# microsoft/MoGe

Hardware: AMD Instinct MI355X
Metric: images/sec (MoGeModel.infer, moge-2-vitl 518x518 fp16) (higher is better)
Workload: dtype f16; 1 GPU; moge-2-vitl infer(): batch 32/GPU x 3x518x518 torch.rand, num_tokens 3600, fp16 weights, synthetic checkpoint (seed 0), inputs resident in HBM, outputs left on device; global_batch=32, parallelism=dp1 (independent shards, one-time RCCL weight broadcast)

## Files before the change

include/moge_hip.h:

```cpp
#ifndef MOGE_HIP_H
#define MOGE_HIP_H

#include <stddef.h>
#include <stdint.h>

#ifdef __cplusplus
extern "C" {
#endif

#define MOGE_ABI_VERSION 5
#define MOGE_MAX_TAPS 8
#define MOGE_LEVELS 5

typedef enum moge_status {
    MOGE_OK = 0,
    MOGE_ERR_INVALID = -1,
    MOGE_ERR_HIP = -2,
    MOGE_ERR_NOT_LOADED = -3,
    MOGE_ERR_MISSING_KEY = -4,
    MOGE_ERR_NONFINITE = -5
} moge_status;

typedef enum moge_precision {
    MOGE_FP32 = 0,
// ... 158 lines not shown
int moge_test_attention(int precision, const float* q, const float* k, const float* v, float* o, int B, int nh, int N, void* stream);
int moge_test_conv3x3(int precision, const float* x, const float* w, const float* bias, float* y, int B, int H, int W,
                      int Cin, int Cout, int relu_in, void* stream);
typedef struct moge_test_conv_args {
    int32_t precision, B, H, W, Cin, Cout;
    int32_t relu_in, act, up2;
    const float* x; const float* w; const float* bias;
    const float* add;
    const float* side; const float* side_w;
    const float* wu; const float* wv; float u0, u1, v0, v1;
    const float* w2; const float* bias2;
    float* y;
    const float* dot_w; int32_t dot_rows;
} moge_test_conv_args;
int moge_test_conv_ex(const moge_test_conv_args* args, void* stream);
typedef struct moge_test_ct3_args {
    int32_t precision, B, H, W, Cin, Cout, no_border;
    const float* x; const float* wt; const float* bt; const float* w3; const float* b3;
    const float* side; const float* side_w;
    const float* wu; const float* wv; float u0, u1, v0, v1;
    float* y;
} moge_test_ct3_args;
int moge_test_ct3(const moge_test_ct3_args* args, void* stream);
int moge_test_convt2x2(int precision, const float* x, const float* w, const float* bias, float* y, int B, int H, int W,
                       int Cin, int Cout, void* stream);
int moge_test_preprocess(const float* image, float* out, int B, int H, int W, int rows, int cols, void* stream);
int moge_test_preprocess_ex(int in_fp16, int out_fp16, const float* image, float* out, int32_t* zero_i32, int B, int H, int W, int rows, int cols, int ldk,
                            int nchw_out, int round16, int aa, int zero_n, void* stream);
int moge_test_resize_bicubic_aa(const float* image, float* out, int B, int H, int W, int OH, int OW, void* stream);
int moge_test_resize_bicubic_aa_ex(int in_fp16, const float* image, float* out, int B, int H, int W, int OH, int OW, int round16, void* stream);
int moge_test_groupnorm_relu(int precision, const float* x, const float* gamma, const float* beta, float* y, int B, int H, int W, int C, int groups, void* stream);
int moge_test_norm_act(int precision, const float* x, const float* gamma, const float* beta, float* y, int B, int H, int W, int C, int groups, int act, int in_place, void* stream);
int moge_test_posembed(const float* pos, float* out, int D, int rows, int cols, void* stream);
int moge_test_posembed_ex(const float* pos, float* out, int D, int rows, int cols, int size_mode, void* stream);
int moge_test_recover(const float* points, const uint8_t* mask, const float* focal_in, int B, int H, int W,
                      float* focal, float* shift, int32_t* status, void* stream);
typedef struct moge_test_head_args {
    int32_t precision, kind, remap, ksize;
    int32_t B, Hd, Wd, C, ld, choff, H, W;
    int32_t n4_below;
    const float* x; const float* w; const float* bias;
    const float* n4; const float* w2;
    float* out;
} moge_test_head_args;
int moge_test_head_final(const moge_test_head_args* args, void* stream);
int moge_test_head_final_dot(int kind, int remap, const float* y, const float* z, int zld, int zoff, const float* bias, float* out, int B, int Hd, int Wd,
// ... 185 lines not shown
```

moge_amd/_lib.py:

```python
from __future__ import annotations

import ctypes as C
import os

import torch

HERE = os.path.dirname(os.path.abspath(__file__))
LIB_PATH = os.path.join(HERE, "lib", "libmoge_hip.so")
EXPERIMENTS_LIB_PATH = os.path.join(HERE, "lib", "experiments", "libmoge_hip.so")

MOGE_MAX_TAPS = 8
MOGE_LEVELS = 5
FP32, FP16, FP16_HALF = 0, 1, 2
HEAD_POINTS, HEAD_NORMAL, HEAD_MASK, HEAD_SCALE = 1, 2, 4, 8
FORCE_PROJECTION, APPLY_MASK = 1, 2
REMAP = {"linear": 0, "sinh": 1, "exp": 2, "sinh_exp": 3}
RESAMPLER = {"conv_transpose": 0, "bilinear": 1, "nearest": 2, "pixel_shuffle": 3}
RES_NORM = {"none": 0, "layer_norm": 1, "group_norm": 2, "instance_norm": 3}
ACTIVATION = {"relu": 0, "leaky_relu": 1, "silu": 2, "elu": 3}
ERR_NONFINITE = -5
KC_NAMES = ["gemm", "attn", "conv", "norm", "pre", "post", "recover", "gemm_pp"]
ABI_VERSION = 5
MESH_MAX_MAPS, MESH_BLOCK_PX, MESH_SCAN_SPAN, MESH_NO_FACES = 8, 1024, 256, -1
MESH_F32, MESH_U8, MESH_UV = 0, 1, 2
# ... 96 lines not shown
    "moge_set_onnx_compatible_mode": (C.c_int, [_vp, _i32]),
    "moge_workspace_bytes": (C.c_int, [_vp, _i32, _i32, _i32, _i32, _i32, C.POINTER(C.c_size_t)]),
    "moge_forward": (C.c_int, [_vp, _vp, _i32, _i32, _i32, _i32, _i32, _i32, C.POINTER(Outputs), _vp]),
    "moge_infer": (C.c_int, [_vp, _vp, _i32, _i32, _i32, _i32, _i32, _i32, _vp, _i32, C.POINTER(Outputs), _vp]),
    "moge_postprocess": (C.c_int, [_vp, _vp, _vp, _vp, _vp, _i32, _i32, _i32, _vp, _i32, C.POINTER(Outputs), _vp]),
    "moge_depth_edge_mask": (C.c_int, [_vp, _vp, _vp, _i32, _i32, _i32, C.c_float, _vp, _vp]),
    "moge_cast_f16": (C.c_int, [_vp, _vp, C.c_int64, _vp]),
    "moge_sync": (C.c_int, [_vp, _vp]),
    "moge_profile_enable": (C.c_int, [_vp, _i32]),
    "moge_profile_read": (C.c_int, [_vp, C.POINTER(Profile), _i32]),
    "moge_debug_tap": (C.c_int, [_vp, C.c_char_p, _vp, _i64, C.POINTER(_i64), _vp]),
    "moge_tune_set": (C.c_int, [C.c_char_p, _i32]),
    "moge_tune_reset": (C.c_int, [C.c_char_p]),
    "moge_tune_value": (C.c_int, [C.c_char_p, C.POINTER(C.c_int)]),
    "moge_test_gemm": (C.c_int, [_i32, _f32p, _f32p, _f32p, _f32p, _i32, _i32, _i32, _i32, _vp]),
    "moge_test_gemm_ex": (C.c_int, [C.POINTER(TestGemmArgs), _vp]),
    "moge_test_gemm_fused_ln": (C.c_int, [_f32p, _f32p, _f32p, _f32p, _f32p, _f32p, _f32p, _f32p, _vp, _i32, _i32, _i32, _vp]),
    "moge_test_layernorm": (C.c_int, [_i32, _f32p, _f32p, _f32p, _f32p, _i32, _i32, _vp]),
    "moge_test_attention": (C.c_int, [_i32, _f32p, _f32p, _f32p, _f32p, _i32, _i32, _i32, _vp]),
    "moge_test_conv3x3": (C.c_int, [_i32, _f32p, _f32p, _f32p, _f32p, _i32, _i32, _i32, _i32, _i32, _i32, _vp]),
    "moge_test_conv_ex": (C.c_int, [C.POINTER(TestConvArgs), _vp]),
    "moge_test_convt2x2": (C.c_int, [_i32, _f32p, _f32p, _f32p, _f32p, _i32, _i32, _i32, _i32, _i32, _vp]),
    "moge_test_ct3": (C.c_int, [C.POINTER(TestCt3Args), _vp]),
    "moge_test_preprocess": (C.c_int, [_f32p, _f32p, _i32, _i32, _i32, _i32, _i32, _vp]),
    "moge_test_preprocess_ex": (C.c_int, [_i32, _i32, _f32p, _f32p, _vp, _i32, _i32, _i32, _i32, _i32, _i32, _i32, _i32, _i32, _i32, _vp]),
    "moge_test_resize_bicubic_aa": (C.c_int, [_f32p, _f32p, _i32, _i32, _i32, _i32, _i32, _vp]),
    "moge_test_resize_bicubic_aa_ex": (C.c_int, [_i32, _f32p, _f32p, _i32, _i32, _i32, _i32, _i32, _i32, _vp]),
    "moge_test_groupnorm_relu": (C.c_int, [_i32, _f32p, _f32p, _f32p, _f32p, _i32, _i32, _i32, _i32, _i32, _vp]),
    "moge_test_norm_act": (C.c_int, [_i32, _f32p, _f32p, _f32p, _f32p, _i32, _i32, _i32, _i32, _i32, _i32, _i32, _vp]),
    "moge_test_posembed": (C.c_int, [_f32p, _f32p, _i32, _i32, _i32, _vp]),
    "moge_test_posembed_ex": (C.c_int, [_f32p, _f32p, _i32, _i32, _i32, _i32, _vp]),
    "moge_test_recover": (C.c_int, [_f32p, _vp, _f32p, _i32, _i32, _i32, _f32p, _f32p, _vp, _vp]),
    "moge_test_head_final": (C.c_int, [C.POINTER(TestHeadArgs), _vp]),
    "moge_test_head_final_dot": (C.c_int, [_i32, _i32, _f32p, _f32p, _i32, _i32, _f32p, _f32p, _i32, _i32, _i32, _i32, _i32, _vp]),
    "moge_test_mlp_layer": (C.c_int, [_f32p, _f32p, _f32p, _f32p, _i32, _i32, _i32, _i32, _vp]),
    "moge_test_layernorm_ex": (C.c_int, [_i32, _i32, _f32p, _f32p, _f32p, _f32p, _f32p, _i32, _i32, _i32, _i32, _i32, _i32, _vp]),
    "moge_test_ln_raw": (C.c_int, [_f32p, _f32p, _f32p, _i32, _i32, _vp]),
    "moge_test_ln_finalize": (C.c_int, [_f32p, _f32p, _i32, _i32, _i32, _vp]),
    "moge_test_fold_ln": (C.c_int, [_f32p, _f32p, _f32p, _f32p, _f32p, _f32p, _f32p, _i32, _i32, _vp]),
    "moge_test_resize_bilinear_uv": (C.c_int, [_i32, _f32p, _f32p, _i32, _i32, _i32, _i32, _i32, _i32, _i32, C.c_float, C.c_float, C.c_float, C.c_float, _vp]),
    "moge_test_u8_ingest": (C.c_int, [_i32, _vp, _f32p, _i32, _i32, _i32, _vp]),
    "moge_align_l1": (C.c_int, [_f32p, _f32p, _f32p, _i32, _i32, C.c_float, _f32p, _f32p, _vp, _vp]),
    "moge_align_l1_anchored": (C.c_int, [_f32p, _f32p, _f32p, _i32, _i32, _i32, _vp, _vp, _i32, C.c_float, _f32p, _f32p, _vp, _vp]),
    "moge_align_trunc_workspace": (C.c_int, [_i32, _i32, C.POINTER(_i64)]),
    "moge_align_trunc": (C.c_int, [_f32p, _f32p, _f32p, _i32, _i32, C.c_float, C.c_float, _vp, _f32p, _f32p, _vp, _vp]),
    "moge_align_trunc_anchored": (C.c_int, [_f32p, _f32p, _f32p, _i32, _i32, _i32, _vp, _vp, _i32, C.c_float, C.c_float, _vp, _f32p, _f32p, _vp, _vp]),
# ... 197 lines not shown
```

moge_amd/csrc/common.h:

```cpp
#pragma once
#include <hip/hip_runtime.h>
#include <stdint.h>
#include <stddef.h>
#include "../../include/moge_hip.h"

typedef _Float16 f16;
typedef unsigned int u32x4 __attribute__((ext_vector_type(4)));
typedef unsigned int u32x2 __attribute__((ext_vector_type(2)));
typedef f16 f16x8 __attribute__((ext_vector_type(8)));
typedef f16 f16x4 __attribute__((ext_vector_type(4)));
typedef f16 f16x2 __attribute__((ext_vector_type(2)));
typedef float f32x2 __attribute__((ext_vector_type(2)));
typedef float f32x4 __attribute__((ext_vector_type(4)));
typedef float f32x16 __attribute__((ext_vector_type(16)));

template <typename T> struct TT;
template <> struct TT<f16> {
    static constexpr int CH = 8;
    static constexpr int PREC = 1;
};
template <> struct TT<float> {
    static constexpr int CH = 4;
    static constexpr int PREC = 0;
};
// ... 194 lines not shown
    static int cus[64] = {};
    int dev = 0;
    if (hipGetDevice(&dev) != hipSuccess) return 256;
    if (dev >= 0 && dev < 64 && cus[dev]) return cus[dev];
    hipDeviceProp_t p;
    const int n = (hipGetDeviceProperties(&p, dev) == hipSuccess && p.multiProcessorCount > 0) ? p.multiProcessorCount : 256;
    if (dev >= 0 && dev < 64) cus[dev] = n;
    return n;
}

template <typename T> int launch_gemm(const GemmArgs& g, int amode, hipStream_t st);
bool gemm_pp_eligible(const GemmArgs& g);
int moge_internal_fail(int code, const char* fmt, ...) __attribute__((format(printf, 2, 3)));
inline int launched(const char* what) {
    const hipError_t e = hipGetLastError();
    return e == hipSuccess ? 0 : moge_internal_fail(MOGE_ERR_HIP, "%s (%s)", what, hipGetErrorString(e));
}
inline unsigned blocks(int64_t n, int per) { return (unsigned)((n + per - 1) / per); }
bool gemm_fuses_ln_finalize(const GemmArgs& g);
bool gemm_runs_pp(const GemmArgs& g);
int launch_gemm_pp(const GemmArgs& g, hipStream_t st);
bool conv_pp_eligible(const GemmArgs& g);
int launch_conv_pp(const GemmArgs& g, hipStream_t st);
struct Ct3Slot { int rowblk, colblk, nterms; int term[13]; };
int launch_ct3_combine(const float* P, const Ct3Slot* slots_dev, int nslots, int Cout, int Cin, void* out, int ld, hipStream_t st);
int launch_ct3_border(const void* in, const void* dw, void* out, int B, int H, int W, int Cin, int Cout, hipStream_t st);
bool conv_rb_eligible(const GemmArgs& g);
int launch_conv_rb(const GemmArgs& g, hipStream_t st);
#include "tune.h"
```

moge_amd/csrc/conv_pp.hip:

```cpp
#include "common.h"

#define CP_GPTR(p) ((const __attribute__((address_space(1))) void*)(p))
__device__ __forceinline__ unsigned cp_opaque(unsigned v) { asm volatile("" : "+v"(v)); return v; }
#define CP_LPTR(p) ((__attribute__((address_space(3))) void*)(p))

namespace {

template <int TW> struct Halo {
    static constexpr int W = TW + 2;
    static constexpr int PX = 18 * W;
    static constexpr int PIECES = (PX + 7) / 8;
    static constexpr int BYTES = PIECES * 1024;
    static constexpr int HPW = (PIECES + 7) / 8;
};

__device__ __forceinline__ u32x4 relu8(u32x4 v) {
#pragma unroll
    for (int i = 0; i < 4; i++) {
        unsigned t = v[i];
        asm("v_pk_max_f16 %0, %0, 0" : "+v"(t));
        v[i] = t;
    }
    return v;
}

template <int N> __device__ __forceinline__ void wait_vm_lgkm() { asm volatile("s_waitcnt vmcnt(%0) lgkmcnt(0)" ::"n"(N) : "memory"); }

template <int BN, int TW, int NH, int EPI>
__global__ __launch_bounds__(512, (BN == 64 && TW == 16 && NH == 1) ? 4 : 2) void conv_pp_kernel(const GemmArgs g) {
    constexpr bool CONVT = (EPI & 2) != 0, HAS_UV = (EPI & 1) != 0, RELU_IN = (EPI & 4) != 0;
    constexpr bool M16 = (EPI & 8) != 0;
    static_assert(!M16 || TW == 16, "16x16x32 path: 16-pixel-wide tiles");
    constexpr bool SIDE_REG = (EPI & 16) != 0;
    constexpr bool DOT = (EPI & 32) != 0;
    static_assert(!DOT || (CONVT && M16 && BN == 128), "fused output conv: the 64 -> 4 x 32 pixel-shuffle resampler");
    constexpr bool CT3 = (EPI & 64) != 0;
    static_assert(!CT3 || (CONVT && M16 && !DOT && !RELU_IN && !SIDE_REG && NH == 2), "fused ConvTranspose2d + 3x3: pixel-shuffle store, 16x16x32 form, two halo buffers");
    constexpr int NTAP = CT3 ? 4 : 9;
    static_assert(!SIDE_REG || (M16 && BN == 64 && NH == 1), "register side input: single-image 64-channel form");
    constexpr int WN = BN / 64, WM = 8 / WN, TM = TW * 16 / 32 / WM, TN = 2;
    constexpr int HALO_W = Halo<TW>::W, HALO_PX = Halo<TW>::PX, HALO_PIECES = Halo<TW>::PIECES, HALO_BYTES = Halo<TW>::BYTES, HPW = Halo<TW>::HPW;
    constexpr int LOG_TW = TW == 16 ? 4 : 5;
    constexpr bool PERSIST = !(BN == 64 && NH == 1);
    constexpr int NWP = BN / 64;
    constexpr int WSLOT = BN * 128;
    constexpr int LDS_W = NH * HALO_BYTES;
    constexpr int WROWS = TM * 32;
    extern __shared__ __attribute__((aligned(16))) char smem[];

    const int tid = threadIdx.x, lane = tid & 63;
    const int wave = __builtin_amdgcn_readfirstlane(tid >> 6);
    const int grp = wave >> 2;
    const int hi = lane >> 5, l31 = lane & 31;
    const int wm = wave / WN, wn = wave % WN;

    const int H = g.H, W = g.W, C = g.C;
    const int tx_n = (W + TW - 1) / TW, ty_n = (H + 15) >> 4;
    const int nbn = g.N / BN;
    int li, cnt, start, wgs_x;
    {
        const int nwg = gridDim.x;
        const int ntiles = PERSIST ? (g.M / (H * W)) * ty_n * tx_n * nbn : nwg;
        const int nx = nwg < 8 ? nwg : 8, xcd = blockIdx.x % nx;
        const int q = ntiles / nx, r = ntiles % nx;
        cnt = q + (xcd < r ? 1 : 0);
        start = xcd * q + min(xcd, r);
        wgs_x = (nwg - xcd + nx - 1) / nx;
        li = blockIdx.x / nx;
    }
    if (li >= cnt) return;
    int b, y0, x0, n0;
    const int nchunks = NH == 1 ? 1 : (C >> 6);
    const int C2 = CT3 ? g.Cout : C;
    const int nside = SIDE_REG ? 1 : ((NH > 1 && g.a2) ? (C2 >> 6) : 0);
    const int nkt1 = nchunks * NTAP;
    const int nkt = nkt1 + nside;

    const int prow = lane >> 3, pch = lane & 7;
    const char* in_b;
    const char* in2_b;
    const char* w_b;
    const char* w2_b;
    unsigned hoff[HPW];
    unsigned hoff2[CT3 ? HPW : 1];
    int sb, sy0, sx0, sn0;
    auto setup = [&](int idx) {
        int prow_t = prow, pch_t = pch;
        if constexpr (PERSIST) asm volatile("" : "+v"(prow_t), "+v"(pch_t));
        const int wgt = start + idx;
        const int bn_ = wgt % nbn;
        int t = wgt / nbn;
        const int tx = t % tx_n; t /= tx_n;
        const int ty = t % ty_n;
        sb = t / ty_n; sy0 = ty * 16; sx0 = tx * TW; sn0 = bn_ * BN;
        in_b = reinterpret_cast<const char*>(g.a) + (size_t)sb * H * W * C * 2;
        in2_b = reinterpret_cast<const char*>(g.a2) + (size_t)sb * H * W * C2 * (CT3 ? 8 : 2);
        w_b = reinterpret_cast<const char*>(g.w) + (size_t)sn0 * g.ldw * 2;
        w2_b = reinterpret_cast<const char*>(g.w2) + (CT3 ? (size_t)0 : (size_t)sn0 * C * 2);
        const int spy = CT3 ? (sn0 / BN) >> 1 : 0, spx = CT3 ? (sn0 / BN) & 1 : 0;
#pragma unroll
        for (int i = 0; i < HPW; i++) {
            int piece = wave + 8 * i;
            piece = piece < HALO_PIECES ? piece : HALO_PIECES - 1;
            int hp = piece * 8 + prow_t;
            const int sw = ((EPI & 8) ? (hp % HALO_W) : ((hp % HALO_W) >> 1)) & 7;
            hp = hp < HALO_PX ? hp : HALO_PX - 1;
            const int hy = hp / HALO_W, hx = hp - hy * HALO_W;
            int yy = sy0 - 1 + hy, xx = sx0 - 1 + hx;
            yy = yy < 0 ? 0 : (yy > H - 1 ? H - 1 : yy);
            xx = xx < 0 ? 0 : (xx > W - 1 ? W - 1 : xx);
            hoff[i] = (unsigned)(((yy * W + xx) * C) * 2 + ((pch_t ^ sw) << 4));
            if constexpr (CT3) hoff2[i] = (unsigned)((((2 * yy + spy) * (2 * W) + 2 * xx + spx) * C2) * 2 + ((pch_t ^ sw) << 4));
        }
    };
    int wrow[NWP];
    unsigned wsw[NWP];
#pragma unroll
    for (int i = 0; i < NWP; i++) {
        wrow[i] = (wave + 8 * i) * 8 + prow;
        wsw[i] = (unsigned)((pch ^ ((wrow[i] >> 1) & 7)) << 4);
    }
    auto issue_halo = [&](int c) {
        char* dst = smem + (c & (NH - 1)) * HALO_BYTES;
        const char* src = uniform_ptr(c < nchunks ? in_b + (size_t)c * 128 : in2_b + (size_t)(c - nchunks) * 128);
        const bool side2 = CT3 && c >= nchunks;
#pragma unroll
        for (int i = 0; i < HPW; i++) {
            int piece = wave + 8 * i;
            piece = piece < HALO_PIECES ? piece : HALO_PIECES - 1;
            unsigned off = hoff[i];
            if constexpr (CT3) off = side2 ? hoff2[i] : off;
            __builtin_amdgcn_global_load_lds(CP_GPTR(src + cp_opaque(off)), CP_LPTR(dst + piece * 1024), 16, 0, 0);
        }
    };
    auto issue_w = [&](int kt) {
        char* dst = smem + LDS_W + (kt & 3) * WSLOT;
        const bool side = kt >= nkt1;
        const int c = CT3 ? kt >> 2 : kt / 9, tap = CT3 ? kt & 3 : kt - c * 9;
        const char* src = uniform_ptr(side ? w2_b + (size_t)(kt - nkt1) * 128 : w_b + ((size_t)tap * C + c * 64) * 2);
        const int rowb = side ? C2 * 2 : g.ldw * 2;
#pragma unroll
        for (int i = 0; i < NWP; i++) {
            const unsigned off = (unsigned)(wrow[i] * rowb) + wsw[i];
            __builtin_amdgcn_global_load_lds(CP_GPTR(src + cp_opaque(off)), CP_LPTR(dst + (wave + 8 * i) * 1024), 16, 0, 0);
        }
    };

    int hp0[TM], hx0[TM];
#pragma unroll
    for (int i = 0; i < TM; i++) {
        const int mp = wm * WROWS + i * 32 + l31;
        hx0[i] = (mp & (TW - 1)) + 1;
        hp0[i] = ((mp >> LOG_TW) + 1) * HALO_W + hx0[i];
    }
    const int sxw = (l31 >> 1) & 7;
    const int w_off = (wn * 64 + l31) * 128 + ((hi ^ sxw) << 4);
    const int l15 = lane & 15, g4 = lane >> 4;
    const int w_off16 = (wn * 64 + l15) * 128 + ((g4 ^ ((l15 >> 1) & 7)) << 4);

    f32x16 acc[TM][TN];
    f32x4 acc16[2 * TM][4];
    const int ntot = nchunks + nside;
    int kt = 0, halo_age = 2;
    int l15t = l15;
    int abase[3][2];
    int tpy = 0;
    auto set_abase = [&]() {
        const bool ph2 = CT3 && BN == 2 * g.Cout;
        const int tpx = CT3 ? (ph2 ? wn : (n0 / BN) & 1) : 0;
        if constexpr (CT3) tpy = ph2 ? (n0 / BN) & 1 : (n0 / BN) >> 1;
#pragma unroll
        for (int d = 0; d < 3; d++) {
            const int hx = l15t + (CT3 ? (d == 2 ? 1 : tpx + d) : d);
            const int a = wm * (2 * TM * HALO_W * 128) + hx * 128 + ((g4 ^ (hx & 7)) << 4);
            abase[d][0] = a; abase[d][1] = a ^ 64;
        }
    };
    u32x4 sidef[SIDE_REG ? 2 * TM : 1][2];
    auto kstep = [&](const char* halo, int dy, int dx, bool first_of_image, int image, bool relu, bool from_regs = false) {
        const char* wsl = smem + LDS_W + (kt & 3) * WSLOT;
        u32x4 af[TM][4], wf[TN][4];
        if constexpr (M16) {
            if (from_regs) {
                if constexpr (SIDE_REG) {
#pragma unroll
                    for (int i = 0; i < 2 * TM; i++)
#pragma unroll
                        for (int ks = 0; ks < 2; ks++) af[i >> 1][(i & 1) * 2 + ks] = sidef[i][ks];
                }
            } else {
#pragma unroll
            for (int i = 0; i < 2 * TM; i++) {
#pragma unroll
                for (int ks = 0; ks < 2; ks++)
                    af[i >> 1][(i & 1) * 2 + ks] = *reinterpret_cast<const u32x4*>(halo + abase[dx + 1][ks] + (i + 1 + dy) * (HALO_W * 128));
            }
            }
#pragma unroll
            for (int j = 0; j < 4; j++)
#pragma unroll
                for (int ks = 0; ks < 2; ks++) wf[j >> 1][(j & 1) * 2 + ks] = *reinterpret_cast<const u32x4*>(wsl + (w_off16 ^ (ks * 64)) + j * 2048);
        } else {
#pragma unroll
        for (int i = 0; i < TM; i++) {
            const int hp = hp0[i] + dy * HALO_W + dx;
// ... 5 lines not shown
        for (int j = 0; j < TN; j++)
#pragma unroll
            for (int ks = 0; ks < 4; ks++) wf[j][ks] = *reinterpret_cast<const u32x4*>(wsl + (w_off ^ (ks * 32)) + j * 4096);
        }
        const bool halo_now = NH > 1 && first_of_image && image + 1 < ntot;
        if (halo_now) { issue_halo(image + 1); halo_age = 0; }
        const int ahead = nkt - 2 - kt;
        if (ahead >= 2) issue_w(kt + 3);
        if (halo_now && image >= nchunks) {
            if (ahead >= 2) wait_vm_lgkm<NWP>();
            else wait_vm_lgkm<0>();
        } else if (NH > 1 && halo_age <= 1) {
            if (ahead >= 2) wait_vm_lgkm<2 * NWP + HPW>();
            else if (ahead == 1) wait_vm_lgkm<NWP + HPW>();
            else wait_vm_lgkm<HPW>();
        } else {
            if (ahead >= 2) wait_vm_lgkm<2 * NWP>();
            else if (ahead == 1) wait_vm_lgkm<NWP>();
            else wait_vm_lgkm<0>();
        }
        halo_age++;
        if constexpr (RELU_IN) {
            if (relu) {
#pragma unroll
                for (int i = 0; i < TM; i++)
#pragma unroll
                    for (int ks = 0; ks < 4; ks++) af[i][ks] = relu8(af[i][ks]);
            }
        }
        __builtin_amdgcn_s_barrier();
        asm volatile("" ::: "memory");
        __builtin_amdgcn_sched_barrier(0);
        __builtin_amdgcn_s_setprio(1);
        if constexpr (M16) {
#pragma unroll
            for (int ks = 0; ks < 2; ks++)
#pragma unroll
                for (int i = 0; i < 2 * TM; i++)
#pragma unroll
                    for (int j = 0; j < 4; j++) mma16<f16>(acc16[i][j], wf[j >> 1][(j & 1) * 2 + ks], af[i >> 1][(i & 1) * 2 + ks]);
        } else {
#pragma unroll
        for (int ks = 0; ks < 4; ks++)
#pragma unroll
            for (int i = 0; i < TM; i++)
#pragma unroll
                for (int j = 0; j < TN; j++) mma_step<f16>(acc[i][j], wf[j][ks], af[i][ks]);
        }
        __builtin_amdgcn_s_setprio(0);
        __builtin_amdgcn_sched_barrier(0);
        asm volatile("" ::: "memory");
        if (!(grp == 1 && kt == nkt - 1)) __builtin_amdgcn_s_barrier();
        asm volatile("" ::: "memory");
        __builtin_amdgcn_sched_barrier(0);
        kt++;
    };
    setup(li);
    if constexpr (SIDE_REG) {
#pragma unroll
        for (int i = 0; i < 2 * TM; i++) {
            int y = sy0 + wm * 2 * TM + i, x = sx0 + l15;
            y = y < H ? y : H - 1; x = x < W ? x : W - 1;
            const char* sp = in2_b + ((size_t)y * W + x) * C * 2 + g4 * 16;
#pragma unroll
            for (int ks = 0; ks < 2; ks++) sidef[i][ks] = *reinterpret_cast<const u32x4*>(sp + ks * 64);
        }
    }
    issue_halo(0);
    bool first = true;
    for (;;) {
    b = sb; y0 = sy0; x0 = sx0; n0 = sn0;
    if constexpr (PERSIST) { asm volatile("" : "+v"(l15t)); if constexpr (M16) set_abase(); }
    else if constexpr (M16) set_abase();
#pragma unroll
    for (int i = 0; i < TM; i++)
#pragma unroll
        for (int j = 0; j < TN; j++)
#pragma unroll
            for (int r = 0; r < 16; r++) acc[i][j][r] = 0.f;
#pragma unroll
    for (int i = 0; i < 2 * TM; i++)
#pragma unroll
        for (int j = 0; j < 4; j++) acc16[i][j] = f32x4{0.f, 0.f, 0.f, 0.f};

    if (!first) {
        asm volatile("s_waitcnt lgkmcnt(0)" ::: "memory");
        __builtin_amdgcn_s_barrier();
        asm volatile("" ::: "memory");
    }
    first = false;
    kt = 0; halo_age = 2;
    issue_w(0);
    issue_w(1);
    issue_w(2);
    wait_vm_lgkm<2 * NWP>();
    __builtin_amdgcn_s_barrier();
    if (grp == 1) __builtin_amdgcn_s_barrier();
    asm volatile("" ::: "memory");
    __builtin_amdgcn_sched_barrier(0);

    for (int c = 0; c < nchunks; c++) {
        const char* halo = smem + (c & (NH - 1)) * HALO_BYTES;
        if constexpr (CT3) {
            const char* hp = halo + tpy * (HALO_W * 128);
#pragma unroll
            for (int tap = 0; tap < 4; tap++) kstep(hp, (tap >> 1) - 1, (tap & 1) - 1, tap == 0, c, true);
        } else {
#pragma unroll
        for (int tap = 0; tap < 9; tap++) kstep(halo, tap / 3 - 1, tap % 3 - 1, tap == 0, c, true);
        }
    }
    if constexpr (SIDE_REG) kstep(smem, 0, 0, false, nchunks, false, true);
    else
    for (int c2 = 0; c2 < nside; c2++) kstep(smem + ((nchunks + c2) & (NH - 1)) * HALO_BYTES, 0, CT3 ? 1 : 0, true, nchunks + c2, false);

    char* R = smem + (PERSIST ? LDS_W : 0) + wave * (WROWS * 128);
    int rr = lane >> 3, cc = lane & 7;
    if constexpr (PERSIST) asm volatile("" : "+v"(rr), "+v"(cc));
    const int nw = n0 + wn * 64;
    const float lo = g.act == ACT_RELU ? 0.f : -3.0e38f;
    const bool has_bias = g.bias != nullptr;
    f16* const outp = reinterpret_cast<f16*>(g.out);
    const f16* const addp = reinterpret_cast<const f16*>(g.add);
    f16x8 addv[WROWS / 8];
    auto load_skip_rows = [&]() {
        if constexpr (!CONVT) {
            if (addp) {
    #pragma unroll
                for (int it = 0; it < WROWS / 8; it++) {
                    const int mp = wm * WROWS + it * 8 + rr;
                    int y = y0 + (mp >> LOG_TW), x = x0 + (mp & (TW - 1));
                    y = y < H ? y : H - 1; x = x < W ? x : W - 1;
                    addv[it] = *reinterpret_cast<const f16x8*>(addp + (((size_t)b * H + y) * W + x) * g.ldadd + nw + cc * 8);
                }
            }
        }
    };
    if constexpr (PERSIST) load_skip_rows();
    u32x4 dota[DOT ? 3 : 1], dotb[DOT ? 2 * TM : 1][2];
    if constexpr (DOT) {
#pragma unroll
        for (int gq = 0; gq < 3; gq++)
            dota[gq] = *reinterpret_cast<const u32x4*>(reinterpret_cast<const char*>(g.dot_tab) + (gq < g.dot_nd ? gq : 0) * 1024 + lane * 16);
    }
    if constexpr (M16) {
        float u0[2 * TM], u1[2 * TM], v0[2 * TM], v1[2 * TM];
        if constexpr (HAS_UV) {
#pragma unroll
            for (int i = 0; i < 2 * TM; i++) {
                int y = y0 + wm * 2 * TM + i, x = x0 + l15;
                y = y < H ? y : H - 1; x = x < W ? x : W - 1;
                if constexpr (CONVT) {
                    u0[i] = linspace_at(g.uv.u0, g.uv.u1, g.uv.ustep, 2 * W, 2 * x);
                    u1[i] = linspace_at(g.uv.u0, g.uv.u1, g.uv.ustep, 2 * W, 2 * x + 1);
                    v0[i] = linspace_at(g.uv.v0, g.uv.v1, g.uv.vstep, 2 * H, 2 * y);
                    v1[i] = linspace_at(g.uv.v0, g.uv.v1, g.uv.vstep, 2 * H, 2 * y + 1);
                } else {
                    u0[i] = u1[i] = linspace_at(g.uv.u0, g.uv.u1, g.uv.ustep, W, x);
                    v0[i] = v1[i] = linspace_at(g.uv.v0, g.uv.v1, g.uv.vstep, H, y);
                }
            }
        }
        f32x4 bvs[4];
#pragma unroll
        for (int jj = 0; jj < 4; jj++) bvs[jj] = *reinterpret_cast<const f32x4*>(g.bias + nw + jj * 16 + 4 * g4);
#pragma unroll
        for (int jj = 0; jj < 4; jj++) {
            const int n = nw + jj * 16 + 4 * g4;
            const f32x4 bv = bvs[jj];
            f32x4 wu = {0.f, 0.f, 0.f, 0.f}, wv = wu;
            int pdy = 0, pdx = 0;
            if constexpr (HAS_UV) {
                int nco = n;
                if constexpr (CONVT) { const int qd = n / g.Cout; nco = n - qd * g.Cout; pdy = qd >> 1; pdx = qd & 1; }
                wu = *reinterpret_cast<const f32x4*>(g.uv.wu + nco);
                wv = *reinterpret_cast<const f32x4*>(g.uv.wv + nco);
            }
#pragma unroll
            for (int i = 0; i < 2 * TM; i++) {
                const int row = i * 16 + l15;
                float v[4];
#pragma unroll
                for (int e = 0; e < 4; e++) v[e] = acc16[i][jj][e] + bv[e];
                if constexpr (HAS_UV) {
                    const float uu = pdx ? u1[i] : u0[i];
                    const float vq = pdy ? v1[i] : v0[i];
#pragma unroll
                    for (int e = 0; e < 4; e++) v[e] += wu[e] * uu + wv[e] * vq;
                }
#pragma unroll
                for (int e = 0; e < 4; e++) v[e] = fmaxf(v[e], lo);
                const f16x4 hv = {(f16)v[0], (f16)v[1], (f16)v[2], (f16)v[3]};
                if constexpr (DOT) {
                    const u32x2 hw = __builtin_bit_cast(u32x2, hv);
                    dotb[i][jj >> 1][(jj & 1) * 2] = hw[0];
                    dotb[i][jj >> 1][(jj & 1) * 2 + 1] = hw[1];
                } else {
                    *reinterpret_cast<f16x4*>(R + row * 128 + ((((jj * 2 + (g4 >> 1)) ^ (row & 7)) << 4) | ((g4 & 1) << 3))) = hv;
                }
            }
        }
        if constexpr (DOT) {
            float* const dout = g.dot_out;
            const int nd4 = 4 * g.dot_nd;
#pragma unroll
            for (int i = 0; i < 2 * TM; i++) {
                const int y = y0 + wm * 2 * TM + i, x = x0 + l15;
                const bool mine = g4 == i && y < H && x < W;
#pragma unroll
                for (int p = 0; p < 2; p++) {
                    const size_t px = ((size_t)b * 2 * H + 2 * y + wn) * (2 * W) + 2 * x + p;
#pragma unroll
                    for (int gq = 0; gq < 3; gq++)
                        if (gq < g.dot_nd) {
                            f32x4 d = {0.f, 0.f, 0.f, 0.f};
                            mma16<f16>(d, dota[gq], dotb[i][p]);
                            if (mine) *reinterpret_cast<f32x4*>(dout + px * nd4 + 4 * gq) = d;
                        }
                }
            }
        }
    } else {
    float u0[TM], u1[TM], v0[TM], v1[TM];
    if constexpr (HAS_UV) {
#pragma unroll
        for (int i = 0; i < TM; i++) {
            const int mp = wm * WROWS + i * 32 + l31;
            int y = y0 + (mp >> LOG_TW), x = x0 + (mp & (TW - 1));
            y = y < H ? y : H - 1; x = x < W ? x : W - 1;
            if constexpr (CONVT) {
                u0[i] = linspace_at(g.uv.u0, g.uv.u1, g.uv.ustep, 2 * W, 2 * x);
// ... 32 lines not shown
                    const float vq = pdy ? v1[i] : v0[i];
#pragma unroll
                    for (int e = 0; e < 4; e++) v[e] += wu[e] * uu + wv[e] * vq;
                }
#pragma unroll
                for (int e = 0; e < 4; e++) v[e] = fmaxf(v[e], lo);
                const f16x4 hv = {(f16)v[0], (f16)v[1], (f16)v[2], (f16)v[3]};
                *reinterpret_cast<f16x4*>(R + row * 128 + ((((j * 4 + q) ^ (row & 7)) << 4) | (hi << 3))) = hv;
            }
        }
    }
    if constexpr (!PERSIST) load_skip_rows();
    bool more = false;
    if constexpr (PERSIST) {
        li += wgs_x;
        more = li < cnt;
        if (more) setup(li);
        __builtin_amdgcn_s_waitcnt(0x0F70);
        if (more) issue_halo(0);
        asm volatile("" ::: "memory");
    }
    if constexpr (!DOT)
#pragma unroll
    for (int it = 0; it < WROWS / 8; it++) {
        const int row = it * 8 + rr;
        const int mp = wm * WROWS + row;
        const int y = y0 + (mp >> LOG_TW), x = x0 + (mp & (TW - 1));
        u32x4 v = *reinterpret_cast<const u32x4*>(R + row * 128 + ((cc ^ (row & 7)) << 4));
        if (y < H && x < W) {
            if constexpr (CONVT) {
                const int n = nw + cc * 8;
                const int qd = n / g.Cout, co = n - qd * g.Cout, pdy = qd >> 1, pdx = qd & 1;
                const size_t idx = ((((size_t)b * 2 * H + 2 * y + pdy) * (2 * W)) + 2 * x + pdx) * g.Cout + co;
                *reinterpret_cast<u32x4*>(outp + idx) = v;
            } else {
                const size_t idx = (((size_t)b * H + y) * W + x) * g.ldc + nw + cc * 8;
                if (addp) {
                    f16x8 h = __builtin_bit_cast(f16x8, v);
                    h += addv[it];
                    v = __builtin_bit_cast(u32x4, h);
                }
                *reinterpret_cast<u32x4*>(outp + idx) = v;
            }
        }
    }
    if (!more) break;
    }
}

template <int BN, int TW, int NH, int EPI>
int launch_conv_cfg(const GemmArgs& g, hipStream_t st) {
    constexpr int smem = NH * Halo<TW>::BYTES + 4 * BN * 128;
    constexpr auto kern = conv_pp_kernel<BN, TW, NH, EPI>;
    if (int rc = set_dyn_lds<kern>(smem)) return rc;
    const long B = (long)g.M / ((long)g.H * g.W);
    const long tiles = B * ((g.H + 15) / 16) * ((g.W + TW - 1) / TW) * (g.N / BN);
    const int ncu = pp_device_cus();
    long slots = (BN == 64 && NH == 1) ? tiles : (long)ncu;
    const long cap = moge_tune_get(TK_CONV_GRID);
    if (cap > 0 && !(BN == 64 && NH == 1)) slots = cap;
    const long grid = tiles < slots ? tiles : slots;
    hipLaunchKernelGGL(kern, dim3((unsigned)grid), dim3(512), smem, st, g);
    return (int)hipGetLastError();
}

}

bool conv_pp_eligible(const GemmArgs& g) {
    if (g.ct3) {
        if ((g.C & 63) || g.K != 4 * g.C || g.ldw != 4 * g.C || !g.bias || g.epi != EPI_CONVT || g.N != 4 * g.Cout) return false;
        if (g.Cout != 128 && g.Cout != 64) return false;
        if (g.add || g.act != ACT_NONE || g.relu_in || g.dot_tab || (g.a2 && !g.w2)) return false;
        if (g.a2 && g.Cout == 64) return false;
        if (g.H < 1 || g.W < 1 || (long)g.M % ((long)g.H * g.W) != 0) return false;
        if ((long)g.H * g.W * g.C * 2 >= (1L << 31) || (long)g.H * g.W * g.Cout * 8 >= (1L << 31)) return false;
// ... 109 lines not shown
            const f32x4 p = red[w][j][lane];
#pragma unroll
            for (int e = 0; e < 4; e++) acc[j][e] += p[e];
        }
    if (!valid) return;
    f16* op = out + (((size_t)b * 2 * H + Y) * (2 * W) + X) * Cout + 4 * g4;
#pragma unroll
    for (int j = 0; j < NJ; j++) {
        f16x4 v = *reinterpret_cast<const f16x4*>(op + j * 16);
        v = f16x4{(f16)((float)v[0] + acc[j][0]), (f16)((float)v[1] + acc[j][1]), (f16)((float)v[2] + acc[j][2]), (f16)((float)v[3] + acc[j][3])};
        *reinterpret_cast<f16x4*>(op + j * 16) = v;
    }
}

int launch_ct3_border(const void* in, const void* dw, void* out, int B, int H, int W, int Cin, int Cout, hipStream_t st) {
    if ((Cin & 31) || (Cout != 128 && Cout != 64) || H < 1 || W < 1) return -1;
    const long mmax = (long)B * ((W > H ? W : H) - 1 > 1 ? (W > H ? W : H) - 1 : 1);
    const dim3 grid((unsigned)((mmax + 15) / 16), 12);
    if (Cout == 128) hipLaunchKernelGGL(ct3_border_kernel<8>, grid, dim3(256), 0, st, (const f16*)in, (const f16*)dw, (f16*)out, B, H, W, Cin);
    else hipLaunchKernelGGL(ct3_border_kernel<4>, grid, dim3(256), 0, st, (const f16*)in, (const f16*)dw, (f16*)out, B, H, W, Cin);
    return (int)hipGetLastError();
}

int launch_conv_pp(const GemmArgs& g, hipStream_t st) {
    if (g.ct3) {
        return g.uv.wu ? launch_conv_cfg<128, 16, 2, 8 | 2 | 64 | 1>(g, st) : launch_conv_cfg<128, 16, 2, 8 | 2 | 64>(g, st);
    }
    const bool side_reg = g.C == 64 && g.N == 64 && g.a2 && !g.uv.wu && !g.relu_in && g.epi == EPI_STORE && moge_tune_get(TK_CONV_SIDE_REG);
    const bool one_image = g.C == 64 && (!g.a2 || side_reg);
    if (g.N == 64) {
#ifdef MOGE_EXPERIMENTS
        if (one_image && g.W >= 32 && moge_tune_get(TK_CONV_TW32)) return launch_conv_epi<64, 32, 1>(g, st);
#endif
        return one_image ? launch_conv_epi<64, 16, 1>(g, st) : launch_conv_epi<64, 16, 2>(g, st);
    }
    return one_image ? launch_conv_epi<128, 16, 1>(g, st) : launch_conv_epi<128, 16, 2>(g, st);
}
```

moge_amd/csrc/tune.h:

```cpp
#pragma once

#define MOGE_TUNE_PRODUCT_KEYS(X) \
    X(ATTN_KERN, 3) \
    X(ATTN_KS, 1) \
    X(ATTN_KS_MID, 0) \
    X(ATTN_Q2_MAX_WGS, -1) \
    X(ATTN_SK_TWICE, 0) \
    X(BATCH_SPLIT, 2) \
    X(CONV_GRID, 0) \
    X(CONV_PP, 1) \
    X(CONV_SIDE_REG, 1) \
    X(FUSE_CT3, 1) \
    X(GEMM_PP, 1) \
    X(GLDS_VARIANT, 2) \
    X(GLDS_SMALL_BLOCKS, 512) \
    X(GLDS_SMALL_NS, 3) \
    X(HEAD_STREAMS, 1) \
    X(HEAD_STREAMS_MAX_B, 1) \
    X(HEAD_PIPE, 1) \
    X(PP_MIN_TILES, 96) \
    X(PP_KERN, -1) \
    X(PP_GRID, 0) \
    X(PP_DBG, 0) \
    X(PP_STAGGER, 0)

#ifdef MOGE_EXPERIMENTS
#define MOGE_TUNE_EXPERIMENT_KEYS(X) \
    X(ATTN_EXP, 0) \
    X(ATTN_VAR, 0) \
    X(ATTN_X, 0) \
    X(ATTN_X_MIN_ROUNDS, 2) \
// ... 28 lines not shown
```

Measured before the change: 254.9 images/s.

## Add 256-output-channel tile form to the persistent conv kernel

Adds a BN=256 variant of the implicit-GEMM 3x3 conv kernel. It splits each 64-channel K chunk into two 32-wide steps and uses 16x16x32 MFMAs, so each wave covers 128 output channels. The goal is to reuse each halo tile across more output channels and cut input re-reads. The variant is selected by default (CONV_BN256=1) for non-ct3 convs with N divisible by 256 when there are enough tiles to fill the CUs. The two-half epilogue it needs adds more registers and a longer store path.

Result: no change. 255.7 images/s (median of 6 runs) (+0.3%).

```diff
diff --git a/include/moge_hip.h b/include/moge_hip.h
--- a/include/moge_hip.h
+++ b/include/moge_hip.h
@@ -204,6 +204,7 @@
     float* y;
 } moge_test_ct3_args;
 int moge_test_ct3(const moge_test_ct3_args* args, void* stream);
+int moge_test_conv_form(int ct3, int B, int H, int W, int Cin, int Cout, int has_side, int has_uv);
 int moge_test_convt2x2(int precision, const float* x, const float* w, const float* bias, float* y, int B, int H, int W,
                        int Cin, int Cout, void* stream);
 int moge_test_preprocess(const float* image, float* out, int B, int H, int W, int rows, int cols, void* stream);
diff --git a/moge_amd/_lib.py b/moge_amd/_lib.py
--- a/moge_amd/_lib.py
+++ b/moge_amd/_lib.py
@@ -142,6 +142,7 @@
     "moge_test_conv_ex": (C.c_int, [C.POINTER(TestConvArgs), _vp]),
     "moge_test_convt2x2": (C.c_int, [_i32, _f32p, _f32p, _f32p, _f32p, _i32, _i32, _i32, _i32, _i32, _vp]),
     "moge_test_ct3": (C.c_int, [C.POINTER(TestCt3Args), _vp]),
+    "moge_test_conv_form": (C.c_int, [_i32, _i32, _i32, _i32, _i32, _i32, _i32, _i32]),
     "moge_test_preprocess": (C.c_int, [_f32p, _f32p, _i32, _i32, _i32, _i32, _i32, _vp]),
     "moge_test_preprocess_ex": (C.c_int, [_i32, _i32, _f32p, _f32p, _vp, _i32, _i32, _i32, _i32, _i32, _i32, _i32, _i32, _i32, _i32, _vp]),
     "moge_test_resize_bicubic_aa": (C.c_int, [_f32p, _f32p, _i32, _i32, _i32, _i32, _i32, _vp]),
diff --git a/moge_amd/csrc/common.h b/moge_amd/csrc/common.h
--- a/moge_amd/csrc/common.h
+++ b/moge_amd/csrc/common.h
@@ -240,6 +240,7 @@
 int launch_gemm_pp(const GemmArgs& g, hipStream_t st);
 bool conv_pp_eligible(const GemmArgs& g);
 int launch_conv_pp(const GemmArgs& g, hipStream_t st);
+int conv_pp_form(const GemmArgs& g);
 struct Ct3Slot { int rowblk, colblk, nterms; int term[13]; };
 int launch_ct3_combine(const float* P, const Ct3Slot* slots_dev, int nslots, int Cout, int Cin, void* out, int ld, hipStream_t st);
 int launch_ct3_border(const void* in, const void* dw, void* out, int B, int H, int W, int Cin, int Cout, hipStream_t st);
diff --git a/moge_amd/csrc/conv_pp.hip b/moge_amd/csrc/conv_pp.hip
--- a/moge_amd/csrc/conv_pp.hip
+++ b/moge_amd/csrc/conv_pp.hip
@@ -38,12 +38,16 @@
     static_assert(!CT3 || (CONVT && M16 && !DOT && !RELU_IN && !SIDE_REG && NH == 2), "fused ConvTranspose2d + 3x3: pixel-shuffle store, 16x16x32 form, two halo buffers");
     constexpr int NTAP = CT3 ? 4 : 9;
     static_assert(!SIDE_REG || (M16 && BN == 64 && NH == 1), "register side input: single-image 64-channel form");
-    constexpr int WN = BN / 64, WM = 8 / WN, TM = TW * 16 / 32 / WM, TN = 2;
+    constexpr bool B256 = BN == 256;
+    static_assert(!B256 || (M16 && TW == 16 && NH == 2 && !DOT && !SIDE_REG), "256-column form: 16x16x32 MFMAs, two halo buffers");
+    constexpr int KS = B256 ? 2 : 1;
+    constexpr int WCH = B256 ? 128 : 64;
+    constexpr int WN = BN / WCH, WM = 8 / WN, TM = TW * 16 / 32 / WM, TN = 2;
     constexpr int HALO_W = Halo<TW>::W, HALO_PX = Halo<TW>::PX, HALO_PIECES = Halo<TW>::PIECES, HALO_BYTES = Halo<TW>::BYTES, HPW = Halo<TW>::HPW;
     constexpr int LOG_TW = TW == 16 ? 4 : 5;
     constexpr bool PERSIST = !(BN == 64 && NH == 1);
-    constexpr int NWP = BN / 64;
-    constexpr int WSLOT = BN * 128;
+    constexpr int NWP = B256 ? 2 : BN / 64;
+    constexpr int WSLOT = B256 ? BN * 64 : BN * 128;
     constexpr int LDS_W = NH * HALO_BYTES;
     constexpr int WROWS = TM * 32;
     extern __shared__ __attribute__((aligned(16))) char smem[];
@@ -73,8 +77,8 @@
     const int nchunks = NH == 1 ? 1 : (C >> 6);
     const int C2 = CT3 ? g.Cout : C;
     const int nside = SIDE_REG ? 1 : ((NH > 1 && g.a2) ? (C2 >> 6) : 0);
-    const int nkt1 = nchunks * NTAP;
-    const int nkt = nkt1 + nside;
+    const int nkt1 = nchunks * NTAP * KS;
+    const int nkt = nkt1 + nside * KS;
 
     const int prow = lane >> 3, pch = lane & 7;
     const char* in_b;
@@ -82,7 +86,8 @@
     const char* w_b;
     const char* w2_b;
     unsigned hoff[HPW];
-    unsigned hoff2[CT3 ? HPW : 1];
+    constexpr bool CT3_SIDE = CT3 && !B256;
+    unsigned hoff2[CT3_SIDE ? HPW : 1];
     int sb, sy0, sx0, sn0;
     auto setup = [&](int idx) {
         int prow_t = prow, pch_t = pch;
@@ -110,38 +115,48 @@
             yy = yy < 0 ? 0 : (yy > H - 1 ? H - 1 : yy);
             xx = xx < 0 ? 0 : (xx > W - 1 ? W - 1 : xx);
             hoff[i] = (unsigned)(((yy * W + xx) * C) * 2 + ((pch_t ^ sw) << 4));
-            if constexpr (CT3) hoff2[i] = (unsigned)((((2 * yy + spy) * (2 * W) + 2 * xx + spx) * C2) * 2 + ((pch_t ^ sw) << 4));
+            if constexpr (CT3_SIDE) hoff2[i] = (unsigned)((((2 * yy + spy) * (2 * W) + 2 * xx + spx) * C2) * 2 + ((pch_t ^ sw) << 4));
         }
     };
     int wrow[NWP];
     unsigned wsw[NWP];
+    int w_off256 = 0;
+    auto set_wlane = [&](int ln) {
+        wrow[0] = wave * 16 + (ln >> 2);
+        wsw[0] = (unsigned)(((ln & 3) ^ ((wrow[0] >> 2) & 3)) << 4);
+        const int r = ln & 15, q = ln >> 4;
+        w_off256 = (wn * 128 + r) * 64 + ((q ^ ((r >> 2) & 3)) << 4);
+    };
 #pragma unroll
     for (int i = 0; i < NWP; i++) {
-        wrow[i] = (wave + 8 * i) * 8 + prow;
-        wsw[i] = (unsigned)((pch ^ ((wrow[i] >> 1) & 7)) << 4);
+        if constexpr (!B256) {
+            wrow[i] = (wave + 8 * i) * 8 + prow;
+            wsw[i] = (unsigned)((pch ^ ((wrow[i] >> 1) & 7)) << 4);
+        }
     }
     auto issue_halo = [&](int c) {
         char* dst = smem + (c & (NH - 1)) * HALO_BYTES;
         const char* src = uniform_ptr(c < nchunks ? in_b + (size_t)c * 128 : in2_b + (size_t)(c - nchunks) * 128);
-        const bool side2 = CT3 && c >= nchunks;
+        const bool side2 = CT3_SIDE && c >= nchunks;
 #pragma unroll
         for (int i = 0; i < HPW; i++) {
             int piece = wave + 8 * i;
             piece = piece < HALO_PIECES ? piece : HALO_PIECES - 1;
             unsigned off = hoff[i];
-            if constexpr (CT3) off = side2 ? hoff2[i] : off;
+            if constexpr (CT3_SIDE) off = side2 ? hoff2[i] : off;
             __builtin_amdgcn_global_load_lds(CP_GPTR(src + cp_opaque(off)), CP_LPTR(dst + piece * 1024), 16, 0, 0);
         }
     };
     auto issue_w = [&](int kt) {
         char* dst = smem + LDS_W + (kt & 3) * WSLOT;
         const bool side = kt >= nkt1;
-        const int c = CT3 ? kt >> 2 : kt / 9, tap = CT3 ? kt & 3 : kt - c * 9;
-        const char* src = uniform_ptr(side ? w2_b + (size_t)(kt - nkt1) * 128 : w_b + ((size_t)tap * C + c * 64) * 2);
+        const int kq = (side ? kt - nkt1 : kt) / KS, half = kt & (KS - 1);
+        const int c = CT3 ? kq >> 2 : kq / 9, tap = CT3 ? kq & 3 : kq - c * 9;
+        const char* src = uniform_ptr((side ? w2_b + (size_t)kq * 128 : w_b + ((size_t)tap * C + c * 64) * 2) + half * 64);
         const int rowb = side ? C2 * 2 : g.ldw * 2;
 #pragma unroll
         for (int i = 0; i < NWP; i++) {
-            const unsigned off = (unsigned)(wrow[i] * rowb) + wsw[i];
+            const unsigned off = B256 ? (unsigned)((wrow[0] + 128 * i) * rowb) + wsw[0] : (unsigned)(wrow[i] * rowb) + wsw[i];
             __builtin_amdgcn_global_load_lds(CP_GPTR(src + cp_opaque(off)), CP_LPTR(dst + (wave + 8 * i) * 1024), 16, 0, 0);
         }
     };
@@ -160,6 +175,7 @@
 
     f32x16 acc[TM][TN];
     f32x4 acc16[2 * TM][4];
+    f32x4 accb[B256 ? 4 : 1][B256 ? 8 : 1];
     const int ntot = nchunks + nside;
     int kt = 0, halo_age = 2;
     int l15t = l15;
@@ -177,10 +193,16 @@
         }
     };
     u32x4 sidef[SIDE_REG ? 2 * TM : 1][2];
-    auto kstep = [&](const char* halo, int dy, int dx, bool first_of_image, int image, bool relu, bool from_regs = false) {
+    auto kstep = [&](const char* halo, int dy, int dx, bool first_of_image, int image, bool relu, bool from_regs = false, int ks256 = 0) {
         const char* wsl = smem + LDS_W + (kt & 3) * WSLOT;
         u32x4 af[TM][4], wf[TN][4];
-        if constexpr (M16) {
+        u32x4 afb[B256 ? 4 : 1], wfb[B256 ? 8 : 1];
+        if constexpr (B256) {
+#pragma unroll
+            for (int i = 0; i < 4; i++) afb[i] = *reinterpret_cast<const u32x4*>(halo + (abase[dx + 1][0] ^ (ks256 * 64)) + (i + 1 + dy) * (HALO_W * 128));
+#pragma unroll
+            for (int j = 0; j < 8; j++) wfb[j] = *reinterpret_cast<const u32x4*>(wsl + w_off256 + j * 1024);
+        } else if constexpr (M16) {
             if (from_regs) {
                 if constexpr (SIDE_REG) {
 #pragma unroll
@@ -232,17 +254,27 @@
         halo_age++;
         if constexpr (RELU_IN) {
             if (relu) {
+                if constexpr (B256) {
+#pragma unroll
+                    for (int i = 0; i < 4; i++) afb[i] = relu8(afb[i]);
+                } else {
 #pragma unroll
                 for (int i = 0; i < TM; i++)
 #pragma unroll
                     for (int ks = 0; ks < 4; ks++) af[i][ks] = relu8(af[i][ks]);
+                }
             }
         }
         __builtin_amdgcn_s_barrier();
         asm volatile("" ::: "memory");
         __builtin_amdgcn_sched_barrier(0);
         __builtin_amdgcn_s_setprio(1);
-        if constexpr (M16) {
+        if constexpr (B256) {
+#pragma unroll
+            for (int i = 0; i < 4; i++)
+#pragma unroll
+                for (int j = 0; j < 8; j++) mma16<f16>(accb[i][j], wfb[j], afb[i]);
+        } else if constexpr (M16) {
 #pragma unroll
             for (int ks = 0; ks < 2; ks++)
 #pragma unroll
@@ -280,6 +312,7 @@
     bool first = true;
     for (;;) {
     b = sb; y0 = sy0; x0 = sx0; n0 = sn0;
+    if constexpr (B256) { int ln = lane; asm volatile("" : "+v"(ln)); set_wlane(ln); }
     if constexpr (PERSIST) { asm volatile("" : "+v"(l15t)); if constexpr (M16) set_abase(); }
     else if constexpr (M16) set_abase();
 #pragma unroll
@@ -292,6 +325,12 @@
     for (int i = 0; i < 2 * TM; i++)
 #pragma unroll
         for (int j = 0; j < 4; j++) acc16[i][j] = f32x4{0.f, 0.f, 0.f, 0.f};
+    if constexpr (B256) {
+#pragma unroll
+        for (int i = 0; i < 4; i++)
+#pragma unroll
+            for (int j = 0; j < 8; j++) accb[i][j] = f32x4{0.f, 0.f, 0.f, 0.f};
+    }
 
     if (!first) {
         asm volatile("s_waitcnt lgkmcnt(0)" ::: "memory");
@@ -314,26 +353,40 @@
         if constexpr (CT3) {
             const char* hp = halo + tpy * (HALO_W * 128);
 #pragma unroll
-            for (int tap = 0; tap < 4; tap++) kstep(hp, (tap >> 1) - 1, (tap & 1) - 1, tap == 0, c, true);
+            for (int tap = 0; tap < 4; tap++)
+#pragma unroll
+                for (int ks = 0; ks < KS; ks++) kstep(hp, (tap >> 1) - 1, (tap & 1) - 1, tap == 0 && ks == 0, c, true, false, ks);
         } else {
 #pragma unroll
-        for (int tap = 0; tap < 9; tap++) kstep(halo, tap / 3 - 1, tap % 3 - 1, tap == 0, c, true);
+        for (int tap = 0; tap < 9; tap++)
+#pragma unroll
+            for (int ks = 0; ks < KS; ks++) kstep(halo, tap / 3 - 1, tap % 3 - 1, tap == 0 && ks == 0, c, true, false, ks);
         }
     }
     if constexpr (SIDE_REG) kstep(smem, 0, 0, false, nchunks, false, true);
     else
-    for (int c2 = 0; c2 < nside; c2++) kstep(smem + ((nchunks + c2) & (NH - 1)) * HALO_BYTES, 0, CT3 ? 1 : 0, true, nchunks + c2, false);
+    for (int c2 = 0; c2 < nside; c2++)
+#pragma unroll
+        for (int ks = 0; ks < KS; ks++) kstep(smem + ((nchunks + c2) & (NH - 1)) * HALO_BYTES, 0, CT3 ? 1 : 0, ks == 0, nchunks + c2, false, false, ks);
 
     char* R = smem + (PERSIST ? LDS_W : 0) + wave * (WROWS * 128);
-    int rr = lane >> 3, cc = lane & 7;
+    int lane_e = lane;
+    if constexpr (B256) asm volatile("" : "+v"(lane_e));
+    const int l15e = lane_e & 15, g4e = lane_e >> 4;
+    int rr = lane_e >> 3, cc = lane_e & 7;
     if constexpr (PERSIST) asm volatile("" : "+v"(rr), "+v"(cc));
-    const int nw = n0 + wn * 64;
+    const int nw = n0 + wn * WCH;
     const float lo = g.act == ACT_RELU ? 0.f : -3.0e38f;
     const bool has_bias = g.bias != nullptr;
     f16* const outp = reinterpret_cast<f16*>(g.out);
     const f16* const addp = reinterpret_cast<const f16*>(g.add);
-    f16x8 addv[WROWS / 8];
-    auto load_skip_rows = [&]() {
+    f16x8 addv[WROWS / 8], addv1[B256 ? WROWS / 8 : 1];
+    f16x4 hold[B256 ? 4 : 1][B256 ? 4 : 1];
+    if constexpr (B256) {
+#pragma unroll
+        for (int it = 0; it < WROWS / 8; it++) addv[it] = addv1[it] = f16x8{0, 0, 0, 0, 0, 0, 0, 0};
+    }
+    auto load_skip_rows = [&](int half = 0) {
         if constexpr (!CONVT) {
             if (addp) {
     #pragma unroll
@@ -341,7 +394,9 @@
                     const int mp = wm * WROWS + it * 8 + rr;
                     int y = y0 + (mp >> LOG_TW), x = x0 + (mp & (TW - 1));
                     y = y < H ? y : H - 1; x = x < W ? x : W - 1;
-                    addv[it] = *reinterpret_cast<const f16x8*>(addp + (((size_t)b * H + y) * W + x) * g.ldadd + nw + cc * 8);
+                    const f16x8 t = *reinterpret_cast<const f16x8*>(addp + (((size_t)b * H + y) * W + x) * g.ldadd + nw + half * 64 + cc * 8);
+                    if (B256 && half) addv1[B256 ? it : 0] = t;
+                    else addv[it] = t;
                 }
             }
         }
@@ -358,7 +413,7 @@
         if constexpr (HAS_UV) {
 #pragma unroll
             for (int i = 0; i < 2 * TM; i++) {
-                int y = y0 + wm * 2 * TM + i, x = x0 + l15;
+                int y = y0 + wm * 2 * TM + i, x = x0 + l15e;
                 y = y < H ? y : H - 1; x = x < W ? x : W - 1;
                 if constexpr (CONVT) {
                     u0[i] = linspace_at(g.uv.u0, g.uv.u1, g.uv.ustep, 2 * W, 2 * x);
@@ -371,13 +426,21 @@
                 }
             }
         }
+        constexpr int NJ = B256 ? 8 : 4;
         f32x4 bvs[4];
 #pragma unroll
-        for (int jj = 0; jj < 4; jj++) bvs[jj] = *reinterpret_cast<const f32x4*>(g.bias + nw + jj * 16 + 4 * g4);
-#pragma unroll
-        for (int jj = 0; jj < 4; jj++) {
-            const int n = nw + jj * 16 + 4 * g4;
-            const f32x4 bv = bvs[jj];
+        for (int jj = 0; jj < 4; jj++) bvs[jj] = *reinterpret_cast<const f32x4*>(g.bias + nw + jj * 16 + 4 * g4e);
+#pragma unroll
+        for (int jj = 0; jj < NJ; jj++) {
+            if constexpr (B256) {
+                if (jj == 4) {
+#pragma unroll
+                    for (int j2 = 0; j2 < 4; j2++) bvs[j2] = *reinterpret_cast<const f32x4*>(g.bias + nw + 64 + j2 * 16 + 4 * g4e);
+                    load_skip_rows(1);
+                }
+            }
+            const int n = nw + jj * 16 + 4 * g4e;
+            const f32x4 bv = bvs[jj & 3];
             f32x4 wu = {0.f, 0.f, 0.f, 0.f}, wv = wu;
             int pdy = 0, pdx = 0;
             if constexpr (HAS_UV) {
@@ -388,10 +451,12 @@
             }
 #pragma unroll
             for (int i = 0; i < 2 * TM; i++) {
-                const int row = i * 16 + l15;
+                const int row = i * 16 + l15e;
                 float v[4];
-#pragma unroll
-                for (int e = 0; e < 4; e++) v[e] = acc16[i][jj][e] + bv[e];
+                f32x4 av;
+                if constexpr (B256) av = accb[i][jj]; else av = acc16[i][jj & 3];
+#pragma unroll
+                for (int e = 0; e < 4; e++) v[e] = av[e] + bv[e];
                 if constexpr (HAS_UV) {
                     const float uu = pdx ? u1[i] : u0[i];
                     const float vq = pdy ? v1[i] : v0[i];
@@ -405,8 +470,10 @@
                     const u32x2 hw = __builtin_bit_cast(u32x2, hv);
                     dotb[i][jj >> 1][(jj & 1) * 2] = hw[0];
                     dotb[i][jj >> 1][(jj & 1) * 2 + 1] = hw[1];
+                } else if (B256 && jj >= 4) {
+                    hold[B256 ? jj - 4 : 0][B256 ? i : 0] = hv;
                 } else {
-                    *reinterpret_cast<f16x4*>(R + row * 128 + ((((jj * 2 + (g4 >> 1)) ^ (row & 7)) << 4) | ((g4 & 1) << 3))) = hv;
+                    *reinterpret_cast<f16x4*>(R + row * 128 + ((((jj * 2 + (g4e >> 1)) ^ (row & 7)) << 4) | ((g4e & 1) << 3))) = hv;
                 }
             }
         }
@@ -415,8 +482,8 @@
             const int nd4 = 4 * g.dot_nd;
 #pragma unroll
             for (int i = 0; i < 2 * TM; i++) {
-                const int y = y0 + wm * 2 * TM + i, x = x0 + l15;
-                const bool mine = g4 == i && y < H && x < W;
+                const int y = y0 + wm * 2 * TM + i, x = x0 + l15e;
+                const bool mine = g4e == i && y < H && x < W;
 #pragma unroll
                 for (int p = 0; p < 2; p++) {
                     const size_t px = ((size_t)b * 2 * H + 2 * y + wn) * (2 * W) + 2 * x + p;
@@ -495,6 +562,19 @@
     }
     if constexpr (!DOT)
 #pragma unroll
+    for (int half = 0; half < (B256 ? 2 : 1); half++) {
+    if constexpr (B256) {
+        if (half) {
+#pragma unroll
+            for (int jj = 0; jj < 4; jj++)
+#pragma unroll
+                for (int i = 0; i < 4; i++) {
+                    const int row = i * 16 + l15e;
+                    *reinterpret_cast<f16x4*>(R + row * 128 + ((((jj * 2 + (g4e >> 1)) ^ (row & 7)) << 4) | ((g4e & 1) << 3))) = hold[B256 ? jj : 0][B256 ? i : 0];
+                }
+        }
+    }
+#pragma unroll
     for (int it = 0; it < WROWS / 8; it++) {
         const int row = it * 8 + rr;
         const int mp = wm * WROWS + row;
@@ -502,20 +582,21 @@
         u32x4 v = *reinterpret_cast<const u32x4*>(R + row * 128 + ((cc ^ (row & 7)) << 4));
         if (y < H && x < W) {
             if constexpr (CONVT) {
-                const int n = nw + cc * 8;
+                const int n = nw + half * 64 + cc * 8;
                 const int qd = n / g.Cout, co = n - qd * g.Cout, pdy = qd >> 1, pdx = qd & 1;
                 const size_t idx = ((((size_t)b * 2 * H + 2 * y + pdy) * (2 * W)) + 2 * x + pdx) * g.Cout + co;
                 *reinterpret_cast<u32x4*>(outp + idx) = v;
             } else {
-                const size_t idx = (((size_t)b * H + y) * W + x) * g.ldc + nw + cc * 8;
+                const size_t idx = (((size_t)b * H + y) * W + x) * g.ldc + nw + half * 64 + cc * 8;
                 if (addp) {
                     f16x8 h = __builtin_bit_cast(f16x8, v);
-                    h += addv[it];
+                    h += (B256 && half) ? addv1[B256 ? it : 0] : addv[it];
                     v = __builtin_bit_cast(u32x4, h);
                 }
                 *reinterpret_cast<u32x4*>(outp + idx) = v;
             }
         }
+    }
     }
     if (!more) break;
     }
@@ -523,7 +604,7 @@
 
 template <int BN, int TW, int NH, int EPI>
 int launch_conv_cfg(const GemmArgs& g, hipStream_t st) {
-    constexpr int smem = NH * Halo<TW>::BYTES + 4 * BN * 128;
+    constexpr int smem = NH * Halo<TW>::BYTES + 4 * (BN == 256 ? BN * 64 : BN * 128);
     constexpr auto kern = conv_pp_kernel<BN, TW, NH, EPI>;
     if (int rc = set_dyn_lds<kern>(smem)) return rc;
     const long B = (long)g.M / ((long)g.H * g.W);
@@ -679,10 +760,24 @@
     return (int)hipGetLastError();
 }
 
+int conv_pp_form(const GemmArgs& g) {
+    const int sw = moge_tune_get(TK_CONV_BN256);
+    const long tiles256 = (long)g.M / ((long)g.H * g.W) * ((g.H + 15) / 16) * ((g.W + 15) / 16) * (g.N / 256);
+    const bool fills = moge_tune_get(TK_CONV_GRID) > 0 || tiles256 >= pp_device_cus();
+    if (g.ct3) return (sw == 2 || sw == 3) && fills && g.Cout == 128 && !g.a2 ? 256 : 128;
+    if (g.N == 64) return 64;
+    const bool bn256 = (sw == 1 || sw == 2) && fills;
+    return bn256 && (g.N & 255) == 0 && g.epi == EPI_STORE && !g.uv.wu && !g.dot_tab ? 256 : 128;
+}
+
 int launch_conv_pp(const GemmArgs& g, hipStream_t st) {
+    const int form = conv_pp_form(g);
     if (g.ct3) {
+        if (form == 256) return g.uv.wu ? launch_conv_cfg<256, 16, 2, 8 | 2 | 64 | 1>(g, st) : launch_conv_cfg<256, 16, 2, 8 | 2 | 64>(g, st);
         return g.uv.wu ? launch_conv_cfg<128, 16, 2, 8 | 2 | 64 | 1>(g, st) : launch_conv_cfg<128, 16, 2, 8 | 2 | 64>(g, st);
     }
+    if (form == 256)
+        return g.relu_in ? launch_conv_cfg<256, 16, 2, 12>(g, st) : launch_conv_cfg<256, 16, 2, 8>(g, st);
     const bool side_reg = g.C == 64 && g.N == 64 && g.a2 && !g.uv.wu && !g.relu_in && g.epi == EPI_STORE && moge_tune_get(TK_CONV_SIDE_REG);
     const bool one_image = g.C == 64 && (!g.a2 || side_reg);
     if (g.N == 64) {
diff --git a/moge_amd/csrc/tune.h b/moge_amd/csrc/tune.h
--- a/moge_amd/csrc/tune.h
+++ b/moge_amd/csrc/tune.h
@@ -7,6 +7,7 @@
     X(ATTN_Q2_MAX_WGS, -1) \
     X(ATTN_SK_TWICE, 0) \
     X(BATCH_SPLIT, 2) \
+    X(CONV_BN256, 1) \
     X(CONV_GRID, 0) \
     X(CONV_PP, 1) \
     X(CONV_SIDE_REG, 1) \
```
